# robflynnyh/long-context-asr

Hardware: AMD Instinct MI355X
Metric: spectrogram-frames/sec (6L/768D, seq=16384) (higher is better)
Workload: dtype bf16; 1 GPU; 6L/768D/6H SConformerXL, seq=16384, rotary theta=1.5M, fwd+CTC+bwd+clip+MADGRAD; per_gpu_batch=128, global_batch=128, seq_len=16384, parallelism=dp1

## Files before the change

### long-context-asr_amd/csrc/common.h

```cpp
#pragma once
#include <hip/hip_runtime.h>
#include <stdint.h>
#include <stdio.h>
#include <stdarg.h>
#include <stdlib.h>
#include <initializer_list>
#include "../../include/sconf.h"

typedef __bf16 bf16;
typedef __attribute__((ext_vector_type(8))) __bf16 bf16x8;
typedef __attribute__((ext_vector_type(4))) __bf16 bf16x4;
typedef __attribute__((ext_vector_type(2))) __bf16 bf16x2;
typedef __attribute__((ext_vector_type(4))) float f32x4;
typedef __attribute__((ext_vector_type(16))) float f32x16;

#define SCONF_API extern "C" __attribute__((visibility("default")))
#include "gfx950.h"

int sconf_set_error(const char* fmt, ...);
#define SCONF_REQUIRE(cond, ...) do { if (!(cond)) return sconf_set_error(__VA_ARGS__); } while (0)
#define SCONF_LAUNCH_OK(name) do { hipError_t e_ = hipGetLastError(); \
    if (e_ != hipSuccess) return sconf_set_error("%s: launch failed: %s", name, hipGetErrorString(e_)); } while (0)

int sconf_stage01_fwd_mfma(const void* x, int x_dtype, const float* w0, const float* b0, const float* wd, const float* bd, void* d1,
// ... 72 lines not shown
    const int w = threadIdx.x >> 6, nw = blockDim.x >> 6;
    __syncthreads();
    if ((threadIdx.x & 63) == 0) sh[w] = v;
    __syncthreads();
    float r = 0.f;
    for (int i = 0; i < nw; ++i) r += sh[i];
    return r;
}
__device__ __forceinline__ float block_max(float v, float* sh) {
    v = wave_max(v);
    const int w = threadIdx.x >> 6, nw = blockDim.x >> 6;
    __syncthreads();
    if ((threadIdx.x & 63) == 0) sh[w] = v;
    __syncthreads();
    float r = -INFINITY;
    for (int i = 0; i < nw; ++i) r = fmaxf(r, sh[i]);
    return r;
}

__device__ __forceinline__ float sigmoidf_(float x) {
    return __builtin_amdgcn_rcpf(1.f + __builtin_amdgcn_exp2f(-1.4426950408889634f * x));
}
__device__ __forceinline__ float siluf_(float x) { return x * sigmoidf_(x); }
__device__ __forceinline__ float dsiluf_(float x) { float s = sigmoidf_(x); return s * (1.f + x * (1.f - s)); }
__device__ __forceinline__ float tanhf_(float x) { return 2.f * sigmoidf_(2.f * x) - 1.f; }
__device__ __forceinline__ float geluf_(float x) {
    const float k = -2.f * 0.7978845608028654f * 1.4426950408889634f;
    const float z = x * (1.f + 0.044715f * x * x);
    return x * __builtin_amdgcn_rcpf(1.f + __builtin_amdgcn_exp2f(k * z));
}
__device__ __forceinline__ void gelu_both(float x, float& g, float& dg) {
    const float c2 = 2.f * 0.7978845608028654f;
    const float x2 = x * x;
    const float z = x * (1.f + 0.044715f * x2);
    const float s = __builtin_amdgcn_rcpf(1.f + __builtin_amdgcn_exp2f(-c2 * 1.4426950408889634f * z));
    g = x * s;
    dg = s + g * (1.f - s) * c2 * (1.f + 3.f * 0.044715f * x2);
}
__device__ __forceinline__ float dgeluf_(float x) {
    const float c2 = 2.f * 0.7978845608028654f;
    const float x2 = x * x;
    const float z = x * (1.f + 0.044715f * x2);
    const float s = __builtin_amdgcn_rcpf(1.f + __builtin_amdgcn_exp2f(-c2 * 1.4426950408889634f * z));
    return s + x * s * (1.f - s) * c2 * (1.f + 3.f * 0.044715f * x2);
}

static inline int cdiv(long a, long b) { return (int)((a + b - 1) / b); }
static inline int64_t round256(int64_t n) { return (n + 255) / 256 * 256; }
static inline int conv_out(long n) { return (int)((n - 1) / 2 + 1); }
static inline int num_cus() {
    static int cus = 0;
    if (!cus) { const int n = sconf_num_cus(); cus = n > 0 ? n : 256; }
    return cus;
}
static inline void lds_limit_once(bool& done, std::initializer_list<const void*> kernels, size_t bytes) {
    if (!done) for (const void* k : kernels) (void)hipFuncSetAttribute(k, hipFuncAttributeMaxDynamicSharedMemorySize, (int)bytes);
    done = true;
}
static inline long env_long(const char* name, long dflt) { const char* e = getenv(name); return e ? atol(e) : dflt; }
static inline bool sub_mfma_off() { const char* e = getenv("SCONF_SUB_MFMA"); return e && e[0] == '0'; }

template <typename T> struct DetSegs { T* out[4]; long off[4]; long n[4]; int k; };

template <typename T>
__global__ __launch_bounds__(1024) void det_reduce_kernel(const T* __restrict__ slab, long rows, long stride, DetSegs<T> s) {
    __shared__ T red[16][64];
    const int lane = threadIdx.x & 63, wv = threadIdx.x >> 6;
    const long col = (long)blockIdx.x * 64 + lane;
    T a = 0;
    if (col < stride) {
#pragma unroll 8
        for (long r = wv; r < rows; r += 16) a += slab[r * stride + col];
    }
    red[wv][lane] = a;
    __syncthreads();
    if (wv == 0 && col < stride) {
        T t = 0;
#pragma unroll
        for (int k = 0; k < 16; ++k) t += red[k][lane];
        for (int i = 0; i < s.k; ++i)
            if (col >= s.off[i] && col < s.off[i] + s.n[i]) s.out[i][col - s.off[i]] += t;
    }
}

template <typename T> T* det_begin(void* ws, int64_t ws_bytes, long rows, long stride, hipStream_t st) {
    const size_t bytes = (size_t)rows * stride * sizeof(T);
    if (!ws || ws_bytes < (int64_t)bytes) return nullptr;
    if (hipMemsetAsync(ws, 0, bytes, st) != hipSuccess) return nullptr;
    return (T*)ws;
}
template <typename T> void det_finish(const T* slab, long rows, long stride, const DetSegs<T>& s, hipStream_t st) {
    hipLaunchKernelGGL(det_reduce_kernel<T>, dim3(cdiv(stride, 64)), dim3(1024), 0, st, slab, rows, stride, s);
}
```

### long-context-asr_amd/csrc/convmod.hip

```cpp
#include "common.h"

namespace {

constexpr int CV = 4;

struct SlabGeo {
    int cg, sl, cpb, spb;
    bool active;
    __device__ __forceinline__ SlabGeo(int CG) {
        cpb = min(64, CG); spb = 256 / cpb;
        const int cgl = threadIdx.x % cpb;
        sl = threadIdx.x / cpb;
        cg = blockIdx.y * cpb + cgl;
        active = cg < CG && sl < spb;
    }
};
template <typename AT>
__device__ __forceinline__ void slab_reduce_add(const float (&v)[CV], const SlabGeo& g, float* sh, AT* out, int d, long det_stride) {
    __syncthreads();
    if (threadIdx.x < g.cpb * g.spb) {
#pragma unroll
        for (int e = 0; e < CV; ++e) sh[g.sl * (g.cpb * CV) + (threadIdx.x % g.cpb) * CV + e] = g.active ? v[e] : 0.f;
    }
    __syncthreads();
    const int nch = g.cpb * CV;
    if ((int)threadIdx.x < nch) {
        const int c = blockIdx.y * nch + threadIdx.x;
        if (c < d) {
            float a = 0.f;
            for (int s_ = 0; s_ < g.spb; ++s_) a += sh[s_ * nch + threadIdx.x];
            atomicAdd(out + (long)blockIdx.x * det_stride + c, (AT)a);
        }
    }
}

template <int K>
__global__ __launch_bounds__(256) void glu_dwconv_fwd_kernel(const bf16* __restrict__ g, const int* __restrict__ len,
                                                             const float* __restrict__ w, const float* __restrict__ bias,
                                                             bf16* __restrict__ h, double* __restrict__ stats,
                                                             int B, int N, int d, int TN, long det_stride) {
    constexpr int P = (K - 1) / 2;
    __shared__ float red[1024];
    const int CG = d / CV, spb = (N + TN - 1) / TN;
    const SlabGeo geo(CG);
    const long slab = (long)blockIdx.x * geo.spb + geo.sl;
    const bool live = geo.active && slab < (long)B * spb;
    const int b = live ? (int)(slab / spb) : 0, n0 = live ? (int)(slab % spb) * TN : 0;
    const int c0 = live ? geo.cg * CV : 0;
    const int L = len ? len[b] : N;
    float wk[K][CV], win[K][CV], bs[CV];
#pragma unroll
    for (int e = 0; e < CV; ++e) {
        bs[e] = bias[c0 + e];
#pragma unroll
        for (int j = 0; j < K; ++j) { wk[j][e] = w[(c0 + e) * K + j]; win[j][e] = 0.f; }
    }
    float s1[CV] = {0.f, 0.f, 0.f, 0.f}, s2[CV] = {0.f, 0.f, 0.f, 0.f};
    const bf16* gb = g + (long)b * N * 2 * d;
    const int nend = live ? min(N, n0 + TN) : n0 - 2 * P;
    const bf16x4 z4 = {(bf16)0.f, (bf16)0.f, (bf16)0.f, (bf16)0.f};
    auto fetch = [&](int t, bf16x4& va, bf16x4& ga) {
        va = z4; ga = z4;
        if (t >= 0 && t < N && t < L) {
            va = *reinterpret_cast<const bf16x4*>(gb + (long)t * 2 * d + c0);
            ga = *reinterpret_cast<const bf16x4*>(gb + (long)t * 2 * d + d + c0);
        }
    };
    bf16x4 cva, cga;
    fetch(n0 - P, cva, cga);
    for (int t = n0 - P; t < nend + P; ++t) {
        bf16x4 nva, nga;
        fetch(t + 1 < nend + P ? t + 1 : -1000000, nva, nga);
#pragma unroll
        for (int j = 0; j < K - 1; ++j)
#pragma unroll
            for (int e = 0; e < CV; ++e) win[j][e] = win[j + 1][e];
#pragma unroll
        for (int e = 0; e < CV; ++e) win[K - 1][e] = (float)cva[e] * sigmoidf_((float)cga[e]);
        const int n = t - P;
        if (n >= n0 && n < nend) {
            float o[CV];
#pragma unroll
            for (int e = 0; e < CV; ++e) {
                float acc = bs[e];
#pragma unroll
                for (int j = 0; j < K; ++j) acc += wk[j][e] * win[j][e];
                const float rr = (float)(bf16)acc;
                o[e] = rr; s1[e] += rr; s2[e] += rr * rr;
            }
            store4(h + ((long)b * N + n) * d + c0, o);
        }
        cva = nva; cga = nga;
    }
    if (stats) {
        slab_reduce_add<double>(s1, geo, red, stats, d, det_stride);
        slab_reduce_add<double>(s2, geo, red, stats + d, d, det_stride);
    }
}

__global__ void brn_finalize_kernel(const double* __restrict__ stats, double count, float* __restrict__ running_mean,
                                    float* __restrict__ running_std, long* __restrict__ nbt, const float* __restrict__ weight,
                                    const float* __restrict__ bias, float* __restrict__ coef, int d, int training,
                                    float eps, float momentum) {
    const int c = blockIdx.x * blockDim.x + threadIdx.x;
    if (c >= d) return;
    const float rm = running_mean[c], rs = running_std[c], w = weight[c], bb = bias[c];
    if (training) {
        const double nb = (double)(*nbt);
        const float rmax = fminf(fmaxf((float)(2.0 / 35000.0 * nb + 25.0 / 35.0), 1.f), 3.f);
        const float dmax = fminf(fmaxf((float)(5.0 / 20000.0 * nb - 25.0 / 20.0), 0.f), 5.f);
        const double mean = stats[c] / count;
        double var = stats[d + c] / count - mean * mean;
        if (var < 0) var = 0;
        const float sigma = (float)sqrt(var), s = sigma + eps;
// ... 122 lines not shown
            if (t < L) {
                r.va = *reinterpret_cast<const bf16x4*>(gbp + (long)t * 2 * d + c0);
                r.ga = *reinterpret_cast<const bf16x4*>(gbp + (long)t * 2 * d + d + c0);
            }
        }
        const int n = t - P;
        if (n >= n0 && n < nend && n < L) {
            r.cva = *reinterpret_cast<const bf16x4*>(gbp + (long)n * 2 * d + c0);
            r.cga = *reinterpret_cast<const bf16x4*>(gbp + (long)n * 2 * d + d + c0);
        }
        return r;
    };
    Raw cur = fetch(n0 - P);
    for (int t = n0 - P; t < nend + P; ++t) {
        const Raw nxt = fetch(t + 1 < nend + P ? t + 1 : -1000000);
#pragma unroll
        for (int j = 0; j < K - 1; ++j)
#pragma unroll
            for (int e = 0; e < CV; ++e) { dhw[j][e] = dhw[j + 1][e]; aw[j][e] = aw[j + 1][e]; }
        if (t >= 0 && t < N) {
#pragma unroll
            for (int e = 0; e < CV; ++e) {
                const float hx = (float)cur.hx[e];
                const float dz = (float)cur.gy[e] * dsiluf_(hx * A[e] + Bc[e]);
                dhw[K - 1][e] = k0[e] * dz - k1[e] - (hx - mean[e]) * is[e] * k2[e];
                aw[K - 1][e] = (t < L) ? (float)cur.va[e] * sigmoidf_((float)cur.ga[e]) : 0.f;
            }
        } else {
#pragma unroll
            for (int e = 0; e < CV; ++e) { dhw[K - 1][e] = 0.f; aw[K - 1][e] = 0.f; }
        }
        const int n = t - P;
        if (n >= n0 && n < nend) {
            float dv[CV], dgt[CV];
#pragma unroll
            for (int e = 0; e < CV; ++e) {
                float acc = 0.f;
                const float dhc = dhw[P][e];
#pragma unroll
                for (int j = 0; j < K; ++j) { acc += wk[j][e] * dhw[K - 1 - j][e]; gw[j][e] += dhc * aw[j][e]; }
                gb[e] += dhc;
                if (n < L) {
                    const float sg = sigmoidf_((float)cur.cga[e]);
                    dv[e] = acc * sg; dgt[e] = acc * (float)cur.cva[e] * sg * (1.f - sg);
                } else { dv[e] = 0.f; dgt[e] = 0.f; }
                sv[e] += dv[e]; sg2[e] += dgt[e];
            }
            bf16* o = dg + ((long)b * N + n) * 2 * d;
            store4(o + c0, dv); store4(o + d + c0, dgt);
        }
        cur = nxt;
    }
    slab_reduce_add<float>(gb, geo, redw, dbias, d, det_stride);
#pragma unroll
    for (int j = 0; j < K; ++j) slab_reduce_add<float>(gw[j], geo, redw, dwt + (long)j * d, d, det_stride);
    if (dgcs) { slab_reduce_add<float>(sv, geo, redw, dgcs, d, det_stride); slab_reduce_add<float>(sg2, geo, redw, dgcs + d, d, det_stride); }
}

int pick_tn(long B, long N, long CG) {
    int TN = 64;
    while (TN > 8 && B * cdiv(N, TN) * CG < 131072) TN >>= 1;
    return TN;
}

}

static dim3 glu_fwd_grid(long B, long N, long d, int& TN) {
    TN = pick_tn(B, N, d / CV);
    const int cpb = (int)std::min<long>(64, d / CV), spbk = 256 / cpb;
    return dim3(cdiv(B * cdiv(N, TN), spbk), cdiv(d / CV, cpb));
}
SCONF_API int64_t sconf_glu_dwconv_fwd_workspace(int64_t B, int64_t N, int64_t d) {
    if (B * N == 0 || d % CV != 0) return 0;
    int TN; return (int64_t)glu_fwd_grid(B, N, d, TN).x * 2 * d * 8;
}
SCONF_API int sconf_glu_dwconv_fwd(const void* g, const int32_t* lengths, const float* w, const float* bias, void* h,
                                   double* stats, void* workspace, int64_t workspace_bytes, int64_t B, int64_t N, int64_t d,
                                   int64_t ksize, hipStream_t stream) {
    SCONF_REQUIRE(d % CV == 0, "sconf_glu_dwconv_fwd: d must be a multiple of 4");
    if (B * N == 0) return 0;
    int TN;
    const dim3 grid = glu_fwd_grid(B, N, d, TN), block(256);
    SCONF_REQUIRE(ksize == 3 || ksize == 5 || ksize == 7 || ksize == 9, "sconf_glu_dwconv_fwd: unsupported kernel size %ld (3,5,7,9)", (long)ksize);
    double* sl = stats ? det_begin<double>(workspace, workspace_bytes, grid.x, 2 * d, stream) : nullptr;
    SCONF_REQUIRE(!stats || sl, "sconf_glu_dwconv_fwd: needs %ld bytes of workspace (sconf_glu_dwconv_fwd_workspace)",
                  (long)sconf_glu_dwconv_fwd_workspace(B, N, d));
#define L(KK) hipLaunchKernelGGL((glu_dwconv_fwd_kernel<KK>), grid, block, 0, stream, (const bf16*)g, lengths, w, bias, (bf16*)h, sl, (int)B, (int)N, (int)d, TN, 2 * d)
    switch (ksize) { case 3: L(3); break; case 5: L(5); break; case 7: L(7); break; default: L(9); break; }
#undef L
    if (stats) det_finish<double>(sl, grid.x, 2 * d, DetSegs<double>{{stats}, {0}, {2 * d}, 1}, stream);
    SCONF_LAUNCH_OK("sconf_glu_dwconv_fwd");
    return 0;
}

SCONF_API int sconf_brn_finalize(const double* stats, int64_t count, float* running_mean, float* running_std,
                                 int64_t* num_batches_tracked, const float* weight, const float* bias, float* coef,
                                 int64_t d, int training, float eps, float momentum, hipStream_t stream) {
    hipLaunchKernelGGL(brn_finalize_kernel, dim3(cdiv(d, 256)), dim3(256), 0, stream, stats, (double)count, running_mean,
                       running_std, (long*)num_batches_tracked, weight, bias, coef, (int)d, training, eps, momentum);
    if (training) hipLaunchKernelGGL(brn_bump_kernel, dim3(1), dim3(64), 0, stream, (long*)num_batches_tracked);
    SCONF_LAUNCH_OK("sconf_brn_finalize");
    return 0;
}

SCONF_API int sconf_affine_silu_fwd(const void* h, const float* coef, void* y, int64_t M, int64_t d, hipStream_t stream) {
    SCONF_REQUIRE(d % 8 == 0, "sconf_affine_silu_fwd: d must be a multiple of 8");
    if (M == 0) return 0;
    const int blocks = (int)std::min<long>(cdiv(M * (d / 8), 256), 8192);
    hipLaunchKernelGGL(affine_silu_fwd_kernel, dim3(blocks), dim3(256), 0, stream, (const bf16*)h, coef, (bf16*)y, (long)M, (int)d);
    SCONF_LAUNCH_OK("sconf_affine_silu_fwd");
    return 0;
}

struct ConvmodBwdGeo { int rpt, cpb, spbk, rrows, TN; dim3 grid; long gst; };
static ConvmodBwdGeo convmod_bwd_geo(long B, long N, long d, long ksize, bool colsum) {
    ConvmodBwdGeo q;
    const long M = B * N;
    const int CG = (int)(d / CV);
    q.rpt = 64;
    while (q.rpt > 8 && cdiv(M, q.rpt) * CG < 131072) q.rpt >>= 1;
    q.cpb = std::min(64, CG); q.spbk = 256 / q.cpb;
    q.rrows = cdiv(cdiv(M, q.rpt), q.spbk);
    q.TN = pick_tn(B, N, CG);
    q.grid = dim3(cdiv(B * cdiv(N, q.TN), q.spbk), cdiv(CG, q.cpb));
    q.gst = d + ksize * d + (colsum ? 2 * d : 0);
    return q;
}
SCONF_API int sconf_convmod_tile_frames(int64_t B, int64_t N, int64_t d) {
    if (B <= 0 || N <= 0 || d <= 0 || d % CV != 0) return -1;
    return pick_tn(B, N, d / CV);
}
SCONF_API int sconf_convmod_bwd_rows_per_thread(int64_t B, int64_t N, int64_t d) {
    if (B <= 0 || N <= 0 || d <= 0 || d % CV != 0) return -1;
    return convmod_bwd_geo(B, N, d, 9, false).rpt;
}
SCONF_API int64_t sconf_convmod_bwd_workspace(int64_t B, int64_t N, int64_t d, int64_t ksize, int colsum) {
    if (B * N == 0 || d % CV != 0) return 0;
    const ConvmodBwdGeo q = convmod_bwd_geo(B, N, d, ksize, colsum != 0);
    return std::max<int64_t>((int64_t)q.rrows * 2 * d * 8, (int64_t)q.grid.x * q.gst * 4);
}
SCONF_API int sconf_convmod_bwd(const void* dy, const void* h, const void* g, const int32_t* lengths, const float* w,
                                const float* brn_weight, const float* coef, double* red, float* bcoef, void* dg,
                                float* dw, float* dbias, float* dbrn_weight, float* dbrn_bias, float* dg_colsum,
                                void* workspace, int64_t workspace_bytes,
                                int64_t B, int64_t N, int64_t d, int64_t ksize, int training, float eps, hipStream_t stream) {
    SCONF_REQUIRE(d % CV == 0, "sconf_convmod_bwd: d must be a multiple of 4");
    const long M = B * N;
    if (M == 0) return 0;
    const int CG = (int)(d / CV);
    SCONF_REQUIRE(ksize == 3 || ksize == 5 || ksize == 7 || ksize == 9, "sconf_convmod_bwd: unsupported kernel size %ld (3,5,7,9)", (long)ksize);
    const ConvmodBwdGeo q = convmod_bwd_geo(B, N, d, ksize, dg_colsum != nullptr);
    const int rpt = q.rpt, cpb = q.cpb, rrows = q.rrows;
    SCONF_REQUIRE(workspace && workspace_bytes >= sconf_convmod_bwd_workspace(B, N, d, ksize, dg_colsum != nullptr),
                  "sconf_convmod_bwd: needs %ld bytes of workspace (sconf_convmod_bwd_workspace)",
                  (long)sconf_convmod_bwd_workspace(B, N, d, ksize, dg_colsum != nullptr));
    double* rsl = det_begin<double>(workspace, workspace_bytes, rrows, 2 * d, stream);
    SCONF_REQUIRE(rsl, "sconf_convmod_bwd: workspace memset failed");
    hipLaunchKernelGGL(brn_bwd_reduce_kernel, dim3(rrows, cdiv(CG, cpb)), dim3(256), 0, stream,
                       (const bf16*)dy, (const bf16*)h, coef, rsl, M, (int)d, rpt, 2 * d);
    det_finish<double>(rsl, rrows, 2 * d, DetSegs<double>{{red}, {0}, {2 * d}, 1}, stream);
    hipLaunchKernelGGL(brn_bwd_finalize_kernel, dim3(cdiv(d, 256)), dim3(256), 0, stream, red, (double)M, coef, brn_weight,
                       bcoef, dbrn_weight, dbrn_bias, (int)d, training, eps);
    const int TN = q.TN;
    const dim3 grid = q.grid, block(256);
    const long gst = q.gst;
    float* gsl = det_begin<float>(workspace, workspace_bytes, grid.x, gst, stream);
    SCONF_REQUIRE(gsl, "sconf_convmod_bwd: workspace memset failed");
#define L(KK) hipLaunchKernelGGL((dwconv_glu_bwd_kernel<KK>), grid, block, 0, stream, (const bf16*)dy, (const bf16*)h, (const bf16*)g, lengths, w, coef, bcoef, (bf16*)dg, gsl + d, gsl, dg_colsum ? gsl + d + ksize * d : nullptr, (int)B, (int)N, (int)d, TN, gst)
    switch (ksize) { case 3: L(3); break; case 5: L(5); break; case 7: L(7); break; default: L(9); break; }
#undef L
    det_finish<float>(gsl, grid.x, gst, DetSegs<float>{{dbias, dw, dg_colsum}, {0, d, d + ksize * d}, {d, ksize * d, dg_colsum ? 2 * d : 0}, dg_colsum ? 3 : 2}, stream);
    SCONF_LAUNCH_OK("sconf_convmod_bwd");
    return 0;
}
```

### long-context-asr_amd/csrc/optim.hip

```cpp
#include "common.h"

namespace {

__global__ __launch_bounds__(256) void sumsq_kernel(const float* __restrict__ g, long n, double* __restrict__ out) {
    __shared__ float sh[16];
    float acc = 0.f;
    long i = ((long)blockIdx.x * 256 + threadIdx.x) * 4;
    const long stride = (long)gridDim.x * 256 * 4;
    for (; i + 4 <= n; i += stride) { float v[4]; load4(g + i, v); acc += v[0] * v[0] + v[1] * v[1] + v[2] * v[2] + v[3] * v[3]; }
    if (i < n) for (long j = i; j < n && j < i + 4; ++j) acc += g[j] * g[j];
    acc = block_sum(acc, sh);
    if (threadIdx.x == 0) out[blockIdx.x] = (double)acc;
}

__global__ __launch_bounds__(256) void madgrad_kernel(float* __restrict__ p, const float* __restrict__ g, float* __restrict__ gss,
                                                      float* __restrict__ s, float* __restrict__ x0, bf16* __restrict__ shadow,
                                                      long n, const double* __restrict__ sumsq, float max_norm, float grad_scale,
                                                      float lr, float ck, float eps, float weight_decay, long k_host,
                                                      const long* __restrict__ k_dev) {
    const long k = k_dev ? *k_dev : k_host;
    const float lamb = lr * sqrtf((float)(k + 1));
    const bool first = k == 0;
    float coef = grad_scale;
    if (sumsq) {
        const double tot = sqrt(*sumsq) * (double)fabsf(grad_scale);
        if (!(tot < INFINITY)) return;
        if (max_norm > 0.f) coef *= fminf(1.f, max_norm / ((float)tot + 1e-6f));
    }
    long i = ((long)blockIdx.x * 256 + threadIdx.x) * 4;
    const long stride = (long)gridDim.x * 256 * 4;
    for (; i + 3 < n; i += stride) {
        float pv[4], gv[4], qv[4], sv[4], xv[4];
        load4(p + i, pv); load4(g + i, gv); load4(gss + i, qv); load4(s + i, sv);
        if (first) {
#pragma unroll
            for (int e = 0; e < 4; ++e) xv[e] = pv[e];
            store4(x0 + i, xv);
        } else load4(x0 + i, xv);
#pragma unroll
        for (int e = 0; e < 4; ++e) {
            float gg = gv[e] * coef;
            if (weight_decay != 0.f) gg += weight_decay * pv[e];
            qv[e] += lamb * gg * gg;
            sv[e] += lamb * gg;
            const float rms = cbrtf(qv[e]) + eps;
            const float z = xv[e] - sv[e] / rms;
            pv[e] = pv[e] * (1.f - ck) + ck * z;
        }
        store4(gss + i, qv); store4(s + i, sv); store4(p + i, pv);
        if (shadow) store4(shadow + i, pv);
    }
    if (i < n) {
        for (long j = i; j < n; ++j) {
            float pv = p[j];
            float gv = g[j] * coef;
            if (weight_decay != 0.f) gv += weight_decay * pv;
            const float q = gss[j] + lamb * gv * gv;
            const float sv = s[j] + lamb * gv;
            const float rms = cbrtf(q) + eps;
            if (first) x0[j] = pv;
            const float z = x0[j] - sv / rms;
            pv = pv * (1.f - ck) + ck * z;
            gss[j] = q; s[j] = sv; p[j] = pv;
            if (shadow) shadow[j] = (bf16)pv;
        }
    }
}

__global__ void madgrad_advance_kernel(long* __restrict__ k_dev, const double* __restrict__ sumsq, float grad_scale) {
    if (sumsq && !(sqrt(*sumsq) * (double)fabsf(grad_scale) < INFINITY)) return;
    *k_dev += 1;
}

}

static int sumsq_blocks(long n) { return (int)std::min<long>(cdiv(n, 1024), 2048); }
SCONF_API int64_t sconf_sumsq_workspace(int64_t n) { return n > 0 ? (int64_t)sumsq_blocks(n) * 8 : 0; }
SCONF_API int sconf_sumsq(const float* g, int64_t n, double* out, void* workspace, int64_t workspace_bytes, hipStream_t stream) {
    if (n == 0) return 0;
    const int blocks = sumsq_blocks(n);
    double* sl = det_begin<double>(workspace, workspace_bytes, blocks, 1, stream);
    SCONF_REQUIRE(sl, "sconf_sumsq: needs %ld bytes of workspace (sconf_sumsq_workspace)", (long)sconf_sumsq_workspace(n));
    hipLaunchKernelGGL(sumsq_kernel, dim3(blocks), dim3(256), 0, stream, g, (long)n, sl);
    det_finish<double>(sl, blocks, 1, DetSegs<double>{{out}, {0}, {1}, 1}, stream);
    SCONF_LAUNCH_OK("sconf_sumsq");
    return 0;
}

SCONF_API int sconf_madgrad_step(float* p, const float* g, float* grad_sum_sq, float* s, float* x0, void* bf16_shadow,
                                 int64_t n, const double* sumsq, float max_norm, float grad_scale, float lr, float momentum,
                                 float eps, float weight_decay, int64_t k, const int64_t* k_dev, hipStream_t stream) {
    if (n == 0) return 0;
    SCONF_REQUIRE(momentum > 0.f && momentum < 1.f, "sconf_madgrad_step: momentum must be in (0,1)");
    if (lr != 0.f) lr = lr + eps;
    const float ck = 1.f - momentum;
    SCONF_REQUIRE((((uintptr_t)p | (uintptr_t)g | (uintptr_t)grad_sum_sq | (uintptr_t)s | (uintptr_t)x0) & 15) == 0 && ((uintptr_t)bf16_shadow & 7) == 0,
                  "sconf_madgrad_step: buffers must be 16-byte aligned");
    const int blocks = (int)std::min<long>(cdiv(n, 1024), 4096);
    hipLaunchKernelGGL(madgrad_kernel, dim3(blocks), dim3(256), 0, stream, p, g, grad_sum_sq, s, x0, (bf16*)bf16_shadow, (long)n,
                       sumsq, max_norm, grad_scale, lr, ck, eps, weight_decay, (long)k, (const long*)k_dev);
    SCONF_LAUNCH_OK("sconf_madgrad_step");
    return 0;
}

SCONF_API int sconf_madgrad_advance(int64_t* k_dev, const double* sumsq, float grad_scale, hipStream_t stream) {
    SCONF_REQUIRE(k_dev != nullptr, "sconf_madgrad_advance: k_dev is null");
    hipLaunchKernelGGL(madgrad_advance_kernel, dim3(1), dim3(1), 0, stream, (long*)k_dev, sumsq, grad_scale);
    SCONF_LAUNCH_OK("sconf_madgrad_advance");
    return 0;
}
```

### long-context-asr_amd/functional.py

```python
from __future__ import annotations

import os

from typing import Optional

import torch
from torch.autograd import Function

from .hip import ops
from .hip import wctc as _wctc

BF16, F32 = torch.bfloat16, torch.float32

class _Shadow:
    __slots__ = ('w', 'rows', 'cols', 'n', 't', 'vn', 'vt', 'regroup')

    def __init__(self, w, regroup=False):
        self.w = w
        self.rows = w.shape[0]; self.cols = w.numel() // max(w.shape[0], 1)
        self.n = None; self.t = None
        self.vn = self.vt = None
        self.regroup = regroup


# ... 507 lines not shown
        out = logits if return_logits else ops.softmax_fwd(logits, True, F32)
        ctx.save_for_backward(nw, nb, wcast_t(wff), bff, hn, out, *saved_norm)
        ctx.cfg = (n_norms, mode, eps, return_logits)
        ctx.P = (nw, nb, wff, bff)
        return out

    @staticmethod
    def backward(ctx, dout):
        n_norms, mode, eps, return_logits = ctx.cfg
        pnw, pnb, pwf, pbf = ctx.P
        sv = ctx.saved_tensors
        nw, nb, wft, bff, hn, out = sv[:6]
        sn = sv[6:]
        dout = dout.contiguous()
        if return_logits:
            dl = ops.cast(dout, BF16)
            dbf = _bgrad(dl, pbf)
        else:
            gbf = _G(pbf)
            dl = ops.softmax_bwd(out, dout, True, BF16, colsum_into=gbf.t)
            dbf = gbf.out()
        dwf = _wgrad(dl, hn, pwf)
        g = ops.gemm(dl, wft, 'nt')
        return _head_norm_bwd(g, sn, nw, pnw, pnb, n_norms, mode, eps) + (dwf, dbf, None, None, None, None)


def decoder_head(x, nw, nb, wff, bff, n_norms=1, mode='layer_norm', eps=1e-5, return_logits=False, prenormed=None):
    return HeadFn.apply(x, prenormed, nw, nb, wff, bff, n_norms, mode, eps, return_logits)


class HeadCTCFn(Function):

    @staticmethod
    def forward(ctx, x, hn_pre, nw, nb, wff, bff, n_norms: int, mode: str, eps: float, B: int, targets, input_lengths, target_lengths, blank: int):
        hn, n_norms, saved_norm = _head_norm_fwd(x, hn_pre, nw, nb, n_norms, mode, eps)
        logits = ops.gemm(hn, wcast(wff), 'nt', bias=bff, out_dtype=F32)
        lg3 = logits.view(B, -1, logits.shape[-1])
        nll, ws = ops.ctc_fwd_logits(lg3, targets, input_lengths, target_lengths, blank)
        ctx.save_for_backward(nw, nb, wcast_t(wff), bff, hn, logits, nll, targets, input_lengths, target_lengths,
                              *[w for w in ws if w is not None], *saved_norm)
        ctx.cfg = (n_norms, mode, eps, B, blank, sum(w is not None for w in ws))
        ctx.P = (nw, nb, wff, bff)
        return nll

    @staticmethod
    def backward(ctx, dnll):
        n_norms, mode, eps, B, blank, nws = ctx.cfg
        pnw, pnb, pwf, pbf = ctx.P
        sv = ctx.saved_tensors
        nw, nb, wft, bff, hn, logits, nll, targets, input_lengths, target_lengths = sv[:10]
        ws = tuple(sv[10:10 + nws]) if nws else (None,) * 5
        sn = sv[10 + nws:]
        gbf = _G(pbf)
        dl = ops.ctc_bwd_logits(logits.view(B, -1, logits.shape[-1]), ws, nll, targets, input_lengths, target_lengths,
                                dnll.contiguous().to(F32), blank, colsum_into=gbf.t if pbf is not None else None)
        dl = dl.view(logits.shape)
        dbf = gbf.out()
        dwf = _wgrad(dl, hn, pwf)
        g = ops.gemm(dl, wft, 'nt')
        return _head_norm_bwd(g, sn, nw, pnw, pnb, n_norms, mode, eps) + (dwf, dbf) + (None,) * 8


def decoder_head_ctc(x, nw, nb, wff, bff, B, targets, input_lengths, target_lengths, blank, n_norms=1, mode='layer_norm', eps=1e-5, prenormed=None,
                     num_labels=None):
    dev = x.device
    _check_ctc_host_args(targets, input_lengths, target_lengths, x.shape[0] // max(B, 1), wff.shape[0] if num_labels is None else num_labels)
    tg, il, tl = _ctc_int_args(dev, targets, input_lengths, target_lengths)
    return HeadCTCFn.apply(x, prenormed, nw, nb, wff, bff, n_norms, mode, eps, B, tg, il, tl, blank)


def _sub_front(audio, w0f, b0, wd1f, bd1, wp1h, bp1):
    d1 = ops.sub_stage01_fwd(audio, w0f, b0, wd1f, bd1)
    return d1, ops.gemm(d1.view(-1, d1.shape[-1]), wp1h, 'nt', bias=bp1).view(d1.shape)


def _sub_tail(pre, woh, bout):
    B, N, Fk, C = pre.shape
    s = ops.sub_silu_transpose(pre.view(B * N, Fk, C))
    return s, ops.gemm(s, woh, 'nt', bias=bout, out_dtype=F32).view(B, N, -1)


def _sub_tail_bwd(dx, pre, s, wot, pwo, pbo):
    B, N, Fk, C = pre.shape
    dx16 = ops.cast(dx.contiguous().view(B * N, -1), BF16)
    ds = ops.gemm(dx16, wot, 'nt')
    dwo = _wgrad(dx16, s, pwo)
    dbo = _bgrad(dx16, pbo)
    return ops.sub_silu_transpose(pre.view(B * N, Fk, C), ds).view(-1, C), dwo, dbo


def _sub_pw_bwd(dpre, xin, wt, pw, pb, gb: Optional[_G] = None):
    dw = _wgrad(dpre, xin.view(-1, xin.shape[-1]), pw)
    db = _bgrad(dpre, pb) if gb is None else gb.out()
    return dw, db, ops.gemm(dpre, wt, 'nt').view(xin.shape)


def _sub_front_bwd(dpre1, gbp1, audio, w0f, b0, wd1f, wp1t, d1, pw0, pb0, pwd1, pbd1, pwp1, pbp1):
    C = d1.shape[-1]
    dwp1, dbp1, dd1 = _sub_pw_bwd(dpre1, d1, wp1t, pwp1, pbp1, gbp1)
    dwd1, dbd1, dw0, db0 = _G(pwd1, (C, 9)), _G(pbd1), _G(pw0, (C, 9)), _G(pb0)
    ops.sub_stage01_bwd_(dd1, audio, w0f, b0, wd1f, dw0.t, db0.t, dwd1.t, dbd1.t)
    return dw0.out(), db0.out(), dwd1.out(), dbd1.out(), dwp1, dbp1


class SubsampleFn(Function):

    @staticmethod
    def forward(ctx, audio, w0, b0, wd1, bd1, wp1, bp1, wd2, bd2, wp2, bp2, wout, bout):
        audio = audio.contiguous()
        C = w0.shape[0]
        w0f, wd1f, wd2f = (t.detach().reshape(C, 9).contiguous() for t in (w0, wd1, wd2))
        wp1h, wp2h, woh = wcast(wp1), wcast(wp2), wcast(wout)
        d1, pre1 = _sub_front(audio, w0f, b0, wd1f, bd1, wp1h, bp1)
        d2 = ops.sub_dwconv_fwd(pre1, wd2f, bd2)
        pre2 = ops.gemm(d2.view(-1, C), wp2h, 'nt', bias=bp2).view(d2.shape)
        s, x = _sub_tail(pre2, woh, bout)
        ctx.save_for_backward(audio, w0f, wd1f, wd2f, wcast_t(wp1), wcast_t(wp2), wcast_t(wout), bp1, bp2, bout, b0, d1, pre1, d2, pre2, s)
        ctx.P = (w0, b0, wd1, bd1, wp1, bp1, wd2, bd2, wp2, bp2, wout, bout)
        return x

    @staticmethod
    def backward(ctx, dx):
        pw0, pb0, pwd1, pbd1, pwp1, pbp1, pwd2, pbd2, pwp2, pbp2, pwo, pbo = ctx.P
        audio, w0f, wd1f, wd2f, wp1t, wp2t, wot, bp1, bp2, bout, b0, d1, pre1, d2, pre2, s = ctx.saved_tensors
        C = d2.shape[-1]
        dpre2, dwo, dbo = _sub_tail_bwd(dx, pre2, s, wot, pwo, pbo)
        dwp2, dbp2, dd2 = _sub_pw_bwd(dpre2, d2, wp2t, pwp2, pbp2)
        dwd2, dbd2 = _G(pwd2, (C, 9)), _G(pbd2)
        gbp1 = _G(pbp1)
        dpre1 = ops.sub_dwconv_bwd(dd2, wd2f, pre1, dwd2.t, dbd2.t, colsum_into=gbp1.t).view(-1, C)
        front = _sub_front_bwd(dpre1, gbp1, audio, w0f, b0, wd1f, wp1t, d1, pw0, pb0, pwd1, pbd1, pwp1, pbp1)
        return (None,) + front + (dwd2.out(), dbd2.out(), dwp2, dbp2, dwo, dbo)


def subsample(audio, w0, b0, wd1, bd1, wp1, bp1, wd2, bd2, wp2, bp2, wout, bout):
    return SubsampleFn.apply(audio, w0, b0, wd1, bd1, wp1, bp1, wd2, bd2, wp2, bp2, wout, bout)


class Subsample4Fn(Function):

    @staticmethod
    def forward(ctx, audio, w0, b0, wd1, bd1, wp1, bp1, wout, bout):
        audio = audio.contiguous()
        C = w0.shape[0]
        w0f, wd1f = (t.detach().reshape(C, 9).contiguous() for t in (w0, wd1))
        wp1h, woh = wcast(wp1), wcast(wout)
        d1, pre1 = _sub_front(audio, w0f, b0, wd1f, bd1, wp1h, bp1)
        s, x = _sub_tail(pre1, woh, bout)
        ctx.save_for_backward(audio, w0f, wd1f, wcast_t(wp1), wcast_t(wout), b0, d1, pre1, s)
        ctx.P = (w0, b0, wd1, bd1, wp1, bp1, wout, bout)
        return x

    @staticmethod
    def backward(ctx, dx):
        pw0, pb0, pwd1, pbd1, pwp1, pbp1, pwo, pbo = ctx.P
        audio, w0f, wd1f, wp1t, wot, b0, d1, pre1, s = ctx.saved_tensors
        dpre1, dwo, dbo = _sub_tail_bwd(dx, pre1, s, wot, pwo, pbo)
        front = _sub_front_bwd(dpre1, None, audio, w0f, b0, wd1f, wp1t, d1, pw0, pb0, pwd1, pbd1, pwp1, pbp1)
        return (None,) + front + (dwo, dbo)


def subsample4(audio, w0, b0, wd1, bd1, wp1, bp1, wout, bout):
    return Subsample4Fn.apply(audio, w0, b0, wd1, bd1, wp1, bp1, wout, bout)


class CTCFn(Function):
    @staticmethod
# ... 89 lines not shown
```

### long-context-asr_amd/hip/ops.py

```python
from __future__ import annotations

import ctypes as C
from typing import Optional, Tuple

import torch

from . import _lib

F32, BF16 = 0, 1
ACT = {'none': 0, 'gelu': 1, 'silu': 2, 'dgelu': 3, 'dsilu': 4, 'gelu_dsave': 5, 'mulaux': 6}
LAYOUT = {'nt': 0, 'nn': 1, 'tn': 2}
NORM_MODE = {'layer_norm': 0, 'rms_norm': 1, 'rms_norm_apex': 2}


def _dt(t: torch.Tensor) -> int:
    if t.dtype == torch.float32:
        return F32
    if t.dtype == torch.bfloat16:
        return BF16
    raise TypeError(f'unsupported dtype {t.dtype}')


def _p(t: Optional[torch.Tensor]):
    return None if t is None else C.c_void_p(t.data_ptr())
# ... 318 lines not shown
    B, N, H, D = q.shape
    if out is None:
        dq = torch.empty(B, N, H, D, dtype=torch.bfloat16, device=q.device)
        dk = torch.empty_like(dq); dv = torch.empty_like(dq)
    else:
        dq, dk, dv = out
    delta = torch.empty(2, B, H, N, dtype=torch.float32, device=q.device)
    sc = float(scale) if scale is not None else D ** -0.5
    cos, sin = rot if rot is not None else (None, None)
    if cos is not None:
        _chk(cos, 'cos', torch.float32); _chk(sin, 'sin', torch.float32)
        if tuple(cos.shape) != (N, D // 2): raise ValueError('rotary tables must be (N, D/2)')
    _lib.call('sconf_attn_bwd', _p(q), _p(k), _p(v), _p(o), _p(dout), _p(lse), _p(delta), _p(dq), _p(dk), _p(dv), _p(lengths),
              B, N, H, D, _strides3(q), _strides3(k), _strides3(v), _strides3(o), _strides3(dout), _strides3(dq), _strides3(dk),
              _strides3(dv), int(window[0]), int(window[1]), sc, _p(cos), _p(sin), _stream())
    return dq, dk, dv


def attn_scores(q: torch.Tensor, k: torch.Tensor, lengths: Optional[torch.Tensor], window=(-1, -1), scale: Optional[float] = None,
                out_dtype: torch.dtype = torch.float32) -> torch.Tensor:
    B, N, H, D = q.shape
    if q.dtype != torch.bfloat16 or k.dtype != torch.bfloat16: raise TypeError('attn_scores: q and k must be bfloat16')
    if tuple(k.shape) != (B, N, H, D): raise ValueError('attn_scores: q and k must have the same (B,N,H,D) shape')
    if lengths is not None: _chk(lengths, 'lengths', torch.int32)
    out = torch.empty(B, H, N, N, dtype=out_dtype, device=q.device)
    sc = float(scale) if scale is not None else D ** -0.5
    _lib.call('sconf_attn_scores', _p(q), _p(k), _p(out), _dt(out), _p(lengths), B, N, H, D, _strides3(q), _strides3(k),
              int(window[0]), int(window[1]), sc, _stream())
    return out


def attn_offset_profile(q: torch.Tensor, k: torch.Tensor, lse: torch.Tensor, lengths: Optional[torch.Tensor], window=(-1, -1),
                        scale: Optional[float] = None) -> torch.Tensor:
    B, N, H, D = q.shape
    if q.dtype != torch.bfloat16 or k.dtype != torch.bfloat16: raise TypeError('attn_offset_profile: q and k must be bfloat16')
    if tuple(k.shape) != (B, N, H, D): raise ValueError('attn_offset_profile: q and k must have the same (B,N,H,D) shape')
    _chk(lse, 'lse', torch.float32)
    if tuple(lse.shape) != (B, H, N): raise ValueError('attn_offset_profile: lse must be (B,H,N)')
    if lengths is not None: _chk(lengths, 'lengths', torch.int32)
    prof = torch.empty(B, H, 2 * N - 1, dtype=torch.float32, device=q.device)
    nws = int(_lib.load().sconf_attn_offset_profile_workspace(B, N, H, int(window[0]), int(window[1])))
    ws = _workspace(nws, q.device)
    sc = float(scale) if scale is not None else D ** -0.5
    _lib.call('sconf_attn_offset_profile', _p(q), _p(k), _p(lse), _p(prof), _p(lengths), B, N, H, D, _strides3(q), _strides3(k),
              int(window[0]), int(window[1]), sc, _p(ws), nws, _stream())
    return prof


def glu_dwconv_fwd(g: torch.Tensor, lengths: Optional[torch.Tensor], w: torch.Tensor, bias: torch.Tensor, B: int, N: int):
    _chk(g, 'g', torch.bfloat16); _chk(w, 'w', torch.float32); _chk(bias, 'bias', torch.float32)
    d = g.shape[-1] // 2
    ks = w.numel() // d
    h = torch.empty(B * N, d, dtype=torch.bfloat16, device=g.device)
    stats = torch.zeros(2, d, dtype=torch.float64, device=g.device)
    nws = int(_lib.load().sconf_glu_dwconv_fwd_workspace(B, N, d))
    ws = _workspace(nws, g.device)
    _lib.call('sconf_glu_dwconv_fwd', _p(g), _p(lengths), _p(w), _p(bias), _p(h), _p(stats), _p(ws), nws, B, N, d, ks, _stream())
    return h, stats


def brn_finalize(stats: torch.Tensor, count: int, running_mean, running_std, num_batches_tracked, weight, bias,
                 training: bool, eps: float = 1e-3, momentum: float = 0.01) -> torch.Tensor:
    d = weight.numel()
    coef = torch.empty(6, d, dtype=torch.float32, device=weight.device)
    _chk(num_batches_tracked, 'num_batches_tracked', torch.int64)
    _lib.call('sconf_brn_finalize', _p(stats), int(count), _p(running_mean), _p(running_std), _p(num_batches_tracked), _p(weight),
              _p(bias), _p(coef), d, int(training), float(eps), float(momentum), _stream())
    return coef


def affine_silu_fwd(h: torch.Tensor, coef: torch.Tensor) -> torch.Tensor:
    _chk(h, 'h', torch.bfloat16)
    d = h.shape[-1]
    y = torch.empty_like(h)
    _lib.call('sconf_affine_silu_fwd', _p(h), _p(coef), _p(y), h.numel() // d, d, _stream())
    return y


def convmod_bwd(dy, h, g, lengths, w, brn_weight, coef, B: int, N: int, training: bool, eps: float,
                dw, dbias, dbrn_weight, dbrn_bias, colsum: bool = False):
    _chk(dy, 'dy', torch.bfloat16); _chk(h, 'h', torch.bfloat16); _chk(g, 'g', torch.bfloat16)
    d = h.shape[-1]; ks = w.numel() // d
    dg = torch.empty(B * N, 2 * d, dtype=torch.bfloat16, device=dy.device)
    red = torch.zeros(2, d, dtype=torch.float64, device=dy.device)
    bcoef = torch.empty(3, d, dtype=torch.float32, device=dy.device)
    dwt = torch.zeros(ks, d, dtype=torch.float32, device=dy.device)
    cs = torch.zeros(2 * d, dtype=torch.float32, device=dy.device) if colsum else None
    nws = int(_lib.load().sconf_convmod_bwd_workspace(B, N, d, ks, int(colsum)))
    ws = _workspace(nws, dy.device)
    _lib.call('sconf_convmod_bwd', _p(dy), _p(h), _p(g), _p(lengths), _p(w), _p(brn_weight), _p(coef), _p(red), _p(bcoef), _p(dg),
              _p(dwt), _p(dbias), _p(dbrn_weight), _p(dbrn_bias), _p(cs), _p(ws), nws, B, N, d, ks, int(training), float(eps), _stream())
    dw.add_(dwt.t())
    return (dg, cs) if colsum else dg


def _half(n: int) -> int:
    return (n - 1) // 2 + 1


def sub_conv0_fwd(x: torch.Tensor, w: torch.Tensor, bias: torch.Tensor) -> torch.Tensor:
    _chk(x, 'x'); _chk(w, 'w', torch.float32)
    B, F, T = x.shape; Cc = w.shape[0]
    y = torch.empty(B, _half(T), _half(F), Cc, dtype=torch.bfloat16, device=x.device)
    _lib.call('sconf_sub_conv0_fwd', _p(x), _dt(x), _p(w), _p(bias), _p(y), B, F, T, Cc, _stream())
    return y


def sub_dwconv_fwd(x: torch.Tensor, w: torch.Tensor, bias: torch.Tensor) -> torch.Tensor:
    _chk(x, 'x', torch.bfloat16)
    B, Ti, Fi, Cc = x.shape
    y = torch.empty(B, _half(Ti), _half(Fi), Cc, dtype=torch.bfloat16, device=x.device)
    _lib.call('sconf_sub_dwconv_fwd', _p(x), _p(w), _p(bias), _p(y), B, Ti, Fi, Cc, _stream())
    return y


def sub_dwconv_bwd(dout: torch.Tensor, w: torch.Tensor, pre_in: torch.Tensor, dw: torch.Tensor, dbias: torch.Tensor,
                   colsum_into: Optional[torch.Tensor] = None) -> torch.Tensor:
    _chk(dout, 'dout', torch.bfloat16); _chk(pre_in, 'pre_in', torch.bfloat16)
    B, Ti, Fi, Cc = pre_in.shape
    dpre = torch.empty_like(pre_in)
    if colsum_into is not None:
        _chk(colsum_into, 'colsum_into', torch.float32)
        if colsum_into.numel() != Cc: raise ValueError('colsum_into must have one element per channel')
    nws = int(_lib.load().sconf_sub_dwconv_bwd_workspace(B, Ti, Fi, Cc, int(colsum_into is not None)))
    ws = _workspace(nws, dout.device)
    _lib.call('sconf_sub_dwconv_bwd', _p(dout), _p(w), _p(pre_in), _p(dpre), _p(dw), _p(dbias), _p(colsum_into), _p(ws), nws,
              B, Ti, Fi, Cc, _stream())
    return dpre


def sub_conv0_bwd_(dpre0: torch.Tensor, x: torch.Tensor, dw: torch.Tensor, dbias: torch.Tensor) -> None:
    _chk(dpre0, 'dpre0', torch.bfloat16); _chk(x, 'x')
    B, F, T = x.shape; Cc = dpre0.shape[-1]
    _lib.call('sconf_sub_conv0_bwd', _p(dpre0), _p(x), _dt(x), _p(dw), _p(dbias), B, F, T, Cc, _stream())


def sub_stage01_fwd(x: torch.Tensor, w0: torch.Tensor, b0: torch.Tensor, wd: torch.Tensor, bd: torch.Tensor) -> torch.Tensor:
    _chk(x, 'x'); _chk(w0, 'w0', torch.float32); _chk(wd, 'wd', torch.float32)
    B, F, T = x.shape; Cc = w0.shape[0]
    d1 = torch.empty(B, _half(_half(T)), _half(_half(F)), Cc, dtype=torch.bfloat16, device=x.device)
    _lib.call('sconf_sub_stage01_fwd', _p(x), _dt(x), _p(w0), _p(b0), _p(wd), _p(bd), _p(d1), B, F, T, Cc, _stream())
    return d1


def sub_stage01_slabs(F: int, C: int, bwd: bool = False) -> int:
    return int(_lib.load().sconf_sub_stage01_slabs(int(F), int(C), int(bool(bwd))))


def sub_stage01_bwd_(dd1: torch.Tensor, x: torch.Tensor, w0, b0, wd, dw0, db0, dwd, dbd) -> None:
    _chk(dd1, 'dd1', torch.bfloat16); _chk(x, 'x')
    B, F, T = x.shape; Cc = dd1.shape[-1]
    nws = int(_lib.load().sconf_sub_stage01_bwd_workspace(B, F, T, Cc))
    ws = _workspace(nws, dd1.device) if nws else None
    _lib.call('sconf_sub_stage01_bwd', _p(dd1), _p(x), _dt(x), _p(w0), _p(b0), _p(wd), _p(dw0), _p(db0), _p(dwd), _p(dbd),
              _p(ws), nws, B, F, T, Cc, _stream())


def sub_silu_transpose(pre: torch.Tensor, ds: Optional[torch.Tensor] = None) -> torch.Tensor:
    _chk(pre, 'pre', torch.bfloat16)
    R, F8, Cc = pre.shape
    if ds is None:
        out = torch.empty(R, Cc * F8, dtype=torch.bfloat16, device=pre.device)
        _lib.call('sconf_sub_silu_transpose', 0, _p(pre), None, _p(out), R, F8, Cc, _stream())
    else:
        _chk(ds, 'ds', torch.bfloat16)
        out = torch.empty_like(pre)
        _lib.call('sconf_sub_silu_transpose', 1, _p(pre), _p(ds), _p(out), R, F8, Cc, _stream())
    return out


# ... 167 lines not shown
```

Measured before the change: 7.128 million spectrogram-frames/sec.

## Skip workspace memsets, store slab partials directly, and add unrolled f64 reduce

Partial-sum slabs now get plain stores instead of atomics, so the per-call hipMemsetAsync of the workspace is skipped for several reductions (glu dwconv stats, convmod bwd, sumsq). A dedicated unrolled f64 deterministic reduce kernel replaces the generic one for doubles. Three zeroed tensors in convmod_bwd are merged into one allocation, and the sub-tail backward reuses a cached bf16 twin instead of casting again. The risk is that any kernel which still accumulates into an unzeroed slab, or leaves some slab rows unwritten, now reads stale data.

```diff
diff --git a/long-context-asr_amd/csrc/common.h b/long-context-asr_amd/csrc/common.h
--- a/long-context-asr_amd/csrc/common.h
+++ b/long-context-asr_amd/csrc/common.h
@@ -178,13 +178,41 @@
             if (col >= s.off[i] && col < s.off[i] + s.n[i]) s.out[i][col - s.off[i]] += t;
     }
 }
-
-template <typename T> T* det_begin(void* ws, int64_t ws_bytes, long rows, long stride, hipStream_t st) {
+constexpr int DET_U = 32;
+template <int U>
+__global__ __launch_bounds__(1024) void det_reduce_f64_kernel(const double* __restrict__ slab, long rows, long stride, DetSegs<double> s) {
+#pragma clang fp reassociate(off)
+    __shared__ double red[16][64];
+    const int lane = threadIdx.x & 63, wv = threadIdx.x >> 6;
+    const long col = (long)blockIdx.x * 64 + lane;
+    double a = 0;
+    if (col < stride) {
+        for (long r = wv; r < rows; r += 16 * U) {
+            double v[U];
+#pragma unroll
+            for (int u = 0; u < U; ++u) v[u] = slab[min(r + 16 * u, rows - 1) * stride + col];
+#pragma unroll
+            for (int u = 0; u < U; ++u) if (r + 16 * u < rows) a += v[u];
+        }
+    }
+    red[wv][lane] = a;
+    __syncthreads();
+    if (wv == 0 && col < stride) {
+        double t = 0;
+#pragma unroll
+        for (int k = 0; k < 16; ++k) t += red[k][lane];
+        for (int i = 0; i < s.k; ++i)
+            if (col >= s.off[i] && col < s.off[i] + s.n[i]) s.out[i][col - s.off[i]] += t;
+    }
+}
+
+template <typename T> T* det_begin(void* ws, int64_t ws_bytes, long rows, long stride, hipStream_t st, bool zero = true) {
     const size_t bytes = (size_t)rows * stride * sizeof(T);
     if (!ws || ws_bytes < (int64_t)bytes) return nullptr;
-    if (hipMemsetAsync(ws, 0, bytes, st) != hipSuccess) return nullptr;
+    if (zero && hipMemsetAsync(ws, 0, bytes, st) != hipSuccess) return nullptr;
     return (T*)ws;
 }
 template <typename T> void det_finish(const T* slab, long rows, long stride, const DetSegs<T>& s, hipStream_t st) {
-    hipLaunchKernelGGL(det_reduce_kernel<T>, dim3(cdiv(stride, 64)), dim3(1024), 0, st, slab, rows, stride, s);
-}
+    if constexpr (sizeof(T) == 8) hipLaunchKernelGGL(det_reduce_f64_kernel<DET_U>, dim3(cdiv(stride, 64)), dim3(1024), 0, st, slab, rows, stride, s);
+    else hipLaunchKernelGGL(det_reduce_kernel<T>, dim3(cdiv(stride, 64)), dim3(1024), 0, st, slab, rows, stride, s);
+}
diff --git a/long-context-asr_amd/csrc/convmod.hip b/long-context-asr_amd/csrc/convmod.hip
--- a/long-context-asr_amd/csrc/convmod.hip
+++ b/long-context-asr_amd/csrc/convmod.hip
@@ -29,7 +29,7 @@
         if (c < d) {
             float a = 0.f;
             for (int s_ = 0; s_ < g.spb; ++s_) a += sh[s_ * nch + threadIdx.x];
-            atomicAdd(out + (long)blockIdx.x * det_stride + c, (AT)a);
+            out[(long)blockIdx.x * det_stride + c] = (AT)a;
         }
     }
 }
@@ -318,7 +318,7 @@
     int TN;
     const dim3 grid = glu_fwd_grid(B, N, d, TN), block(256);
     SCONF_REQUIRE(ksize == 3 || ksize == 5 || ksize == 7 || ksize == 9, "sconf_glu_dwconv_fwd: unsupported kernel size %ld (3,5,7,9)", (long)ksize);
-    double* sl = stats ? det_begin<double>(workspace, workspace_bytes, grid.x, 2 * d, stream) : nullptr;
+    double* sl = stats ? det_begin<double>(workspace, workspace_bytes, grid.x, 2 * d, stream, false) : nullptr;
     SCONF_REQUIRE(!stats || sl, "sconf_glu_dwconv_fwd: needs %ld bytes of workspace (sconf_glu_dwconv_fwd_workspace)",
                   (long)sconf_glu_dwconv_fwd_workspace(B, N, d));
 #define L(KK) hipLaunchKernelGGL((glu_dwconv_fwd_kernel<KK>), grid, block, 0, stream, (const bf16*)g, lengths, w, bias, (bf16*)h, sl, (int)B, (int)N, (int)d, TN, 2 * d)
@@ -390,8 +390,8 @@
     SCONF_REQUIRE(workspace && workspace_bytes >= sconf_convmod_bwd_workspace(B, N, d, ksize, dg_colsum != nullptr),
                   "sconf_convmod_bwd: needs %ld bytes of workspace (sconf_convmod_bwd_workspace)",
                   (long)sconf_convmod_bwd_workspace(B, N, d, ksize, dg_colsum != nullptr));
-    double* rsl = det_begin<double>(workspace, workspace_bytes, rrows, 2 * d, stream);
-    SCONF_REQUIRE(rsl, "sconf_convmod_bwd: workspace memset failed");
+    double* rsl = det_begin<double>(workspace, workspace_bytes, rrows, 2 * d, stream, false);
+    SCONF_REQUIRE(rsl, "sconf_convmod_bwd: workspace too small");
     hipLaunchKernelGGL(brn_bwd_reduce_kernel, dim3(rrows, cdiv(CG, cpb)), dim3(256), 0, stream,
                        (const bf16*)dy, (const bf16*)h, coef, rsl, M, (int)d, rpt, 2 * d);
     det_finish<double>(rsl, rrows, 2 * d, DetSegs<double>{{red}, {0}, {2 * d}, 1}, stream);
@@ -400,8 +400,8 @@
     const int TN = q.TN;
     const dim3 grid = q.grid, block(256);
     const long gst = q.gst;
-    float* gsl = det_begin<float>(workspace, workspace_bytes, grid.x, gst, stream);
-    SCONF_REQUIRE(gsl, "sconf_convmod_bwd: workspace memset failed");
+    float* gsl = det_begin<float>(workspace, workspace_bytes, grid.x, gst, stream, false);
+    SCONF_REQUIRE(gsl, "sconf_convmod_bwd: workspace too small");
 #define L(KK) hipLaunchKernelGGL((dwconv_glu_bwd_kernel<KK>), grid, block, 0, stream, (const bf16*)dy, (const bf16*)h, (const bf16*)g, lengths, w, coef, bcoef, (bf16*)dg, gsl + d, gsl, dg_colsum ? gsl + d + ksize * d : nullptr, (int)B, (int)N, (int)d, TN, gst)
     switch (ksize) { case 3: L(3); break; case 5: L(5); break; case 7: L(7); break; default: L(9); break; }
 #undef L
diff --git a/long-context-asr_amd/csrc/optim.hip b/long-context-asr_amd/csrc/optim.hip
--- a/long-context-asr_amd/csrc/optim.hip
+++ b/long-context-asr_amd/csrc/optim.hip
@@ -79,7 +79,7 @@
 SCONF_API int sconf_sumsq(const float* g, int64_t n, double* out, void* workspace, int64_t workspace_bytes, hipStream_t stream) {
     if (n == 0) return 0;
     const int blocks = sumsq_blocks(n);
-    double* sl = det_begin<double>(workspace, workspace_bytes, blocks, 1, stream);
+    double* sl = det_begin<double>(workspace, workspace_bytes, blocks, 1, stream, false);
     SCONF_REQUIRE(sl, "sconf_sumsq: needs %ld bytes of workspace (sconf_sumsq_workspace)", (long)sconf_sumsq_workspace(n));
     hipLaunchKernelGGL(sumsq_kernel, dim3(blocks), dim3(256), 0, stream, g, (long)n, sl);
     det_finish<double>(sl, blocks, 1, DetSegs<double>{{out}, {0}, {1}, 1}, stream);
diff --git a/long-context-asr_amd/functional.py b/long-context-asr_amd/functional.py
--- a/long-context-asr_amd/functional.py
+++ b/long-context-asr_amd/functional.py
@@ -613,7 +613,8 @@
 
 def _sub_tail_bwd(dx, pre, s, wot, pwo, pbo):
     B, N, Fk, C = pre.shape
-    dx16 = ops.cast(dx.contiguous().view(B * N, -1), BF16)
+    dx16, _ = _take_twin(dx.contiguous())
+    dx16 = dx16.view(B * N, -1)
     ds = ops.gemm(dx16, wot, 'nt')
     dwo = _wgrad(dx16, s, pwo)
     dbo = _bgrad(dx16, pbo)
diff --git a/long-context-asr_amd/hip/ops.py b/long-context-asr_amd/hip/ops.py
--- a/long-context-asr_amd/hip/ops.py
+++ b/long-context-asr_amd/hip/ops.py
@@ -424,10 +424,11 @@
     _chk(dy, 'dy', torch.bfloat16); _chk(h, 'h', torch.bfloat16); _chk(g, 'g', torch.bfloat16)
     d = h.shape[-1]; ks = w.numel() // d
     dg = torch.empty(B * N, 2 * d, dtype=torch.bfloat16, device=dy.device)
-    red = torch.zeros(2, d, dtype=torch.float64, device=dy.device)
+    z = torch.zeros((4 + ks + (2 if colsum else 0)) * d, dtype=torch.float32, device=dy.device)
+    red = z[:4 * d].view(torch.float64).view(2, d)
     bcoef = torch.empty(3, d, dtype=torch.float32, device=dy.device)
-    dwt = torch.zeros(ks, d, dtype=torch.float32, device=dy.device)
-    cs = torch.zeros(2 * d, dtype=torch.float32, device=dy.device) if colsum else None
+    dwt = z[4 * d:(4 + ks) * d].view(ks, d)
+    cs = z[(4 + ks) * d:] if colsum else None
     nws = int(_lib.load().sconf_convmod_bwd_workspace(B, N, d, ks, int(colsum)))
     ws = _workspace(nws, dy.device)
     _lib.call('sconf_convmod_bwd', _p(dy), _p(h), _p(g), _p(lengths), _p(w), _p(brn_weight), _p(coef), _p(red), _p(bcoef), _p(dg),
```

Result: no change. 7.144 million spectrogram-frames/sec, median of 4 (+0.2%).
